# rubiruchi/ofdm_uhd

Measured on AMD Instinct MI355X. Metric: OFDM symbols/sec (TX+loopback RX) @ N_fft=512; packet CRC pass rate, higher is better.
Workload: dtype f32; 1 GPU; N_fft=512, occ=200, QPSK, CP=128, synthetic AWGN channel (BASELINE configs[1]); payload_bytes=1026, symbols_per_packet=22, streams=1, iq_buffers=1, parallelism=independent streams, 1 per GPU

## Files before the change

include/ofdm_hip.h:

```cpp
#ifndef OFDM_HIP_H
#define OFDM_HIP_H

#include <stddef.h>
#include <stdint.h>

#ifdef __cplusplus
extern "C" {
#endif

#define OFDM_ABI_VERSION 6

#define OFDM_MAX_FFT 4096
#define OFDM_MAX_CARRIER_HEX 1024
#define OFDM_MAX_TAPS 512
#define OFDM_MAX_ARITY 256
#define OFDM_MASK_LEN 4096
#define OFDM_MAX_PKT_LEN 4096

enum {
  OFDM_OK = 0,
  OFDM_E_INVAL = -1,
  OFDM_E_NOMEM = -2,
  OFDM_E_CAPACITY = -3,
  OFDM_E_HIP = -4,
// ... 456 lines not shown
int ofdm_ldpc_payload_len(uint32_t coded_len, uint32_t *payload_len);
int ofdm_ldpc_coded_len_rate(uint32_t rate, uint32_t payload_len, uint32_t *coded_len);
int ofdm_ldpc_payload_len_rate(uint32_t rate, uint32_t coded_len, uint32_t *payload_len);
int ofdm_ldpc_encode(ofdm_handle *h, const ofdm_ldpc_cfg *cfg, const uint8_t *payloads, const uint64_t *payload_off,
                     const uint32_t *payload_len, int nblk, uint8_t *coded, uint64_t coded_cap, uint64_t *coded_off);
int ofdm_ldpc_decode(ofdm_handle *h, const ofdm_ldpc_cfg *cfg, const uint8_t *coded, const uint64_t *coded_off,
                     const uint32_t *coded_len, int nblk, uint8_t *payloads, uint64_t payload_cap, uint64_t *payload_off,
                     uint8_t *ok, uint32_t *corrected, uint8_t *iters, uint32_t *cw_failed);
int ofdm_ldpc_decode_soft(ofdm_handle *h, const ofdm_ldpc_cfg *cfg, const int8_t *soft, const uint64_t *soft_off,
                          const uint32_t *coded_len, int nblk, uint8_t *payloads, uint64_t payload_cap,
                          uint64_t *payload_off, uint8_t *ok, uint32_t *corrected, uint8_t *iters, uint32_t *cw_failed);
int ofdm_rx_ldpc_decode_soft(ofdm_handle *h, const ofdm_ldpc_cfg *cfg, uint8_t *payloads, uint64_t payload_cap,
                             uint64_t *payload_off, uint8_t *ok, uint32_t *corrected, uint8_t *iters, uint32_t *cw_failed,
                             int max_pkts, int *n);
int ofdm_ldpc_last_ms(const ofdm_handle *h, double *ms);

int ofdm_rx_set_origin(ofdm_handle *h, uint64_t first_sample_index);
int ofdm_rx_submit(ofdm_handle *h, const ofdm_c32 *iq, uint64_t nsamples);
int ofdm_rx_packet_pos(ofdm_handle *h, uint64_t *pos, int cap, int *n);
int ofdm_rx_nco_state(ofdm_handle *h, uint64_t *flags, uint64_t *phase, double *step, uint8_t *swallowed,
                      int cap, int *n);
int ofdm_rx_set_flag_history(ofdm_handle *h, int enable, int n, const int64_t *flags, const double *steps,
                             const uint8_t *swallowed, int64_t trust_after, int64_t pred_flag, uint64_t pred_phase, double pred_step);

enum {
  OFDM_TAP_TX_PACKETS = 0,
  OFDM_TAP_TX_FREQ = 1,
  OFDM_TAP_RX_CHAN_FILT = 2,
  OFDM_TAP_RX_METRIC = 3,
  OFDM_TAP_RX_PEAKS = 4,
  OFDM_TAP_RX_ANGLES = 5,
  OFDM_TAP_RX_FRAMES = 6,
  OFDM_TAP_RX_FFT = 7,
  OFDM_TAP_RX_ACQ = 8,
  OFDM_TAP_RX_SINK = 9,
  OFDM_TAP_RX_PACKETS = 10,
  OFDM_TAP_TX_MAPPER = 11,
  OFDM_TAP_TX_IFFT = 12,
  OFDM_TAP_RX_SAMPLER = 13,
  OFDM_TAP_RX_SIGMIX = 14,
  OFDM_TAP_RX_NCO = 15,
  OFDM_TAP_RX_PRESEL = 16,
  OFDM_TAP_RX_DEMAPPED = 17,
  OFDM_TAP_RX_RUN_AVG = 18,
  OFDM_TAP_COUNT = 19
};
// ... 27 lines not shown
```

ofdm_uhd_amd/_abi.py:

```python
import ctypes as C
import os

OFDM_ABI_VERSION = 6
OFDM_MAX_FFT = 4096
OFDM_MAX_TAPS = 512
OFDM_MAX_ARITY = 256
OFDM_MASK_LEN = 4096
OFDM_MAX_PKT_LEN = 4096
OFDM_MAX_CARRIER_HEX = 1024
OFDM_DDC_MAX_TAPS = 1024
OFDM_DDC_BANK_MAX_LINKS = 8
OFDM_RESAMP_MAX_TAPS = 1024
OFDM_RESAMP_BANK_MAX_LINKS = 8
OFDM_DUC_MAX_TAPS = 1024
OFDM_DUC_BANK_MAX_LINKS = 8
OFDM_TX_RESAMP_MAX_TAPS = 1024
OFDM_TX_RESAMP_BANK_MAX_LINKS = 8
OFDM_PFB_MAX_CHANNELS = 64
OFDM_PFB_MAX_TAPS = 1024
OFDM_MULTIPATH_MAX_PATHS = 16
OFDM_MULTIPATH_MAX_TONES = 4
OFDM_MULTIPATH_MAX_DELAY = 1023
OFDM_FEC_MAX_PAYLOAD = 2040
OFDM_FEC_MAX_CODED = 4090
# ... 64 lines not shown
        ("fixed_freq_offset", C.c_float),
        ("reserved0", C.c_uint32),
    ]


class ofdm_chan(C.Structure):
    _fields_ = [
        ("sigma", C.c_float),
        ("cfo", C.c_float),
        ("seed", C.c_uint64),
        ("stream_id", C.c_uint64),
        ("lead_samples", C.c_uint64),
        ("tail_samples", C.c_uint64),
    ]


class ofdm_stats(C.Structure):
    _fields_ = [(n, C.c_uint64) for n in (
        "symbols", "samples", "peaks", "frames", "headers_ok", "packets", "crc_ok",
        "chained_frames", "overflow")]

    def as_dict(self):
        return {n: int(getattr(self, n)) for n, _ in self._fields_}


class ofdm_sense_cfg(C.Structure):
    _fields_ = [
        ("struct_size", C.c_uint32),
        ("fft_size", C.c_uint32),
        ("tune_delay", C.c_uint32),
        ("dwell_delay", C.c_uint32),
        ("avg_msgs", C.c_uint32),
        ("skip_msgs", C.c_uint32),
        ("threshold", C.c_double),
        ("window", C.c_float * OFDM_SENSE_MAX_FFT),
    ]


class ofdm_pkt_quality(C.Structure):
    _fields_ = [
        ("flag", C.c_uint64),
        ("first_symbol", C.c_uint32),
        ("nsym", C.c_uint32),
        ("ncarriers", C.c_uint32),
        ("coarse", C.c_int32),
        ("cfo_bins", C.c_float),
# ... 201 lines not shown
    "ofdm_set_rx_iq_format", "ofdm_set_tx_iq_format",
    "ofdm_set_ddc", "ofdm_ddc_reset", "ofdm_ddc_count", "ofdm_ddc", "ofdm_ddc_taps", "ofdm_ddc_last_ms",
    "ofdm_set_duc", "ofdm_duc_reset", "ofdm_duc", "ofdm_duc_last_ms",
    "ofdm_set_ddc_bank", "ofdm_ddc_bank_reset", "ofdm_ddc_bank_count", "ofdm_ddc_bank", "ofdm_ddc_bank_taps",
    "ofdm_ddc_bank_last_ms",
    "ofdm_set_resamp", "ofdm_resamp_reset", "ofdm_resamp_count", "ofdm_resamp", "ofdm_resamp_taps", "ofdm_resamp_last_ms",
    "ofdm_set_resamp_bank", "ofdm_resamp_bank_reset", "ofdm_resamp_bank_count", "ofdm_resamp_bank", "ofdm_resamp_bank_taps",
    "ofdm_resamp_bank_last_ms",
    "ofdm_set_tx_resamp", "ofdm_tx_resamp_reset", "ofdm_tx_resamp_count", "ofdm_tx_resamp", "ofdm_tx_resamp_last_ms",
    "ofdm_set_pfb", "ofdm_pfb_reset", "ofdm_pfb_count", "ofdm_pfb", "ofdm_pfb_last_ms",
    "ofdm_set_pfb_synth", "ofdm_pfb_synth_reset", "ofdm_pfb_synth", "ofdm_pfb_synth_last_ms",
    "ofdm_set_duc_bank", "ofdm_duc_bank_reset", "ofdm_duc_bank", "ofdm_duc_bank_taps", "ofdm_duc_bank_last_ms",
    "ofdm_set_tx_resamp_bank", "ofdm_tx_resamp_bank_reset", "ofdm_tx_resamp_bank_count", "ofdm_tx_resamp_bank",
    "ofdm_tx_resamp_bank_taps", "ofdm_tx_resamp_bank_last_ms",
    "ofdm_set_multipath", "ofdm_multipath_reset", "ofdm_multipath", "ofdm_multipath_last_ms",
    "ofdm_fec_coded_len", "ofdm_fec_payload_len", "ofdm_fec_encode", "ofdm_fec_decode", "ofdm_fec_decode_soft",
    "ofdm_fec_last_ms", "ofdm_fec_coded_len_rate", "ofdm_fec_payload_len_rate", "ofdm_fec_punct_last_ms",
    "ofdm_set_rx_soft", "ofdm_rx_soft", "ofdm_rx_fec_decode_soft", "ofdm_rx_soft_last_ms",
    "ofdm_fec_decode_rel", "ofdm_fec_decode_soft_rel", "ofdm_rx_fec_decode_soft_rel",
    "ofdm_rs_coded_len", "ofdm_rs_payload_len", "ofdm_rs_encode", "ofdm_rs_decode", "ofdm_rs_last_ms",
    "ofdm_rs_decode_rel", "ofdm_rs_rel_from_soft", "ofdm_rs_rel_last_ms",
    "ofdm_ldpc_coded_len", "ofdm_ldpc_payload_len", "ofdm_ldpc_encode", "ofdm_ldpc_decode", "ofdm_ldpc_decode_soft",
    "ofdm_rx_ldpc_decode_soft", "ofdm_ldpc_last_ms", "ofdm_ldpc_coded_len_rate", "ofdm_ldpc_payload_len_rate",
)

_LIB = None
LIB_PATH = os.environ.get("OFDM_HIP_LIB") or os.path.join(os.path.dirname(os.path.abspath(__file__)), "csrc",
                                                         "libofdm_hip.so")


def _declare(lib):
    vp, u8p, u32p, u64p = C.c_void_p, C.c_void_p, C.POINTER(C.c_uint32), C.POINTER(C.c_uint64)
    H = C.c_void_p
    lib.ofdm_abi_version.restype = C.c_int
    lib.ofdm_device_count.restype = C.c_int
    lib.ofdm_create.argtypes = [C.POINTER(ofdm_cfg), C.POINTER(H)]
    lib.ofdm_destroy.argtypes = [H]
    lib.ofdm_destroy.restype = None
    lib.ofdm_last_error.argtypes = [H]
    lib.ofdm_last_error.restype = C.c_char_p
    lib.ofdm_set_stream.argtypes = [H, vp]
    lib.ofdm_set_tx_amplitude.argtypes = [H, C.c_float]
    lib.ofdm_set_carrier_map.argtypes = [H, C.c_char_p]
    lib.ofdm_set_channel.argtypes = [H, C.POINTER(ofdm_chan)]
    lib.ofdm_framed_len.argtypes = [H, C.c_uint32, u32p]
    lib.ofdm_make_packets.argtypes = [H, u8p, u64p, u32p, C.c_int, u8p, C.c_uint64, u64p]
# ... 95 lines not shown
    lib.ofdm_ldpc_coded_len_rate.argtypes = [C.c_uint32, C.c_uint32, u32p]
    lib.ofdm_ldpc_payload_len_rate.argtypes = [C.c_uint32, C.c_uint32, u32p]
    lib.ofdm_ldpc_encode.argtypes = [H, LC, u8p, u64p, u32p, C.c_int, u8p, C.c_uint64, u64p]
    lib.ofdm_ldpc_decode.argtypes = [H, LC, u8p, u64p, u32p, C.c_int, u8p, C.c_uint64, u64p, vp, u32p, vp, u32p]
    lib.ofdm_ldpc_decode_soft.argtypes = lib.ofdm_ldpc_decode.argtypes
    lib.ofdm_rx_ldpc_decode_soft.argtypes = [H, LC, u8p, C.c_uint64, u64p, vp, u32p, vp, u32p, C.c_int, C.POINTER(C.c_int)]
    lib.ofdm_ldpc_last_ms.argtypes = [H, C.POINTER(C.c_double)]
    lib.ofdm_set_taps.argtypes = [H, C.c_uint32]
    lib.ofdm_tap.argtypes = [H, C.c_int, vp, C.c_uint64, u64p]
    lib.ofdm_prof_enable.argtypes = [H, C.c_int]
    lib.ofdm_prof_reset.argtypes = [H]
    lib.ofdm_prof_get.argtypes = [H, C.c_int, C.POINTER(C.c_double), u64p]
    lib.ofdm_kernel_name.argtypes = [C.c_int]
    lib.ofdm_kernel_name.restype = C.c_char_p
    SC = C.POINTER(ofdm_sense_cfg)
    lib.ofdm_sense_count.argtypes = [SC, C.c_uint64, u64p, u64p]
    lib.ofdm_sense.argtypes = [H, SC, vp, C.c_uint64, vp, C.c_uint64, vp, vp, vp, C.c_uint64, u64p, u64p]
    lib.ofdm_sense_decide.argtypes = [H, SC, vp, C.c_uint64, vp, vp, vp, C.c_uint64, u64p]
    lib.ofdm_set_rx_sense.argtypes = [H, SC]
    lib.ofdm_rx_sense_result.argtypes = [H, vp, C.c_uint64, vp, vp, vp, C.c_uint64, u64p, u64p]
    lib.ofdm_rx_packet_pos.argtypes = [H, vp, C.c_int, C.POINTER(C.c_int)]
    lib.ofdm_rx_nco_state.argtypes = [H, vp, vp, vp, vp, C.c_int, C.POINTER(C.c_int)]
    lib.ofdm_rx_set_origin.argtypes = [H, C.c_uint64]
    lib.ofdm_rx_snr.argtypes = [H, C.POINTER(C.c_float)]
    lib.ofdm_set_rx_quality.argtypes = [H, C.c_int]
    lib.ofdm_rx_quality.argtypes = [H, vp, C.c_int, C.POINTER(C.c_int)]
    lib.ofdm_set_rx_csi.argtypes = [H, C.c_int]
    lib.ofdm_rx_csi.argtypes = [H, C.c_int, C.c_int, vp, vp, vp, vp, C.POINTER(C.c_int)]
    lib.ofdm_rx_csi_summary.argtypes = [H, C.c_int, u32p, vp, vp, vp, vp, vp]
    lib.ofdm_rx_submit.argtypes = [H, C.c_void_p, C.c_uint64]
    lib.ofdm_rx_set_flag_history.argtypes = [H, C.c_int, C.c_int, vp, vp, vp, C.c_int64, C.c_int64, C.c_uint64, C.c_double]
    lib.ofdm_sense_device_msgs.argtypes = [H, C.POINTER(C.c_void_p), u64p, u32p]
    lib.ofdm_sense_redecide.argtypes = [H, SC]
    for name in EXPORTS:
        fn = getattr(lib, name)
        if fn.restype is C.c_int and name not in ("ofdm_abi_version", "ofdm_device_count"):
            pass
    return lib


def _preload_hip_runtime():
    try:
        import importlib.util
        spec = importlib.util.find_spec("torch")
        if spec is None or not spec.origin:
            return
# ... 22 lines not shown
```

ofdm_uhd_amd/csrc/engine_rx.inc:

```

template <typename T>
static int dev_excl_scan(ofdm_handle* h, const T* d_in, uint64_t n, T* d_out, T* d_total) {
  const uint64_t nb = (n + SCAN_BLOCK - 1) / SCAN_BLOCK;
  HIPCHK(h, h->rx.partial.ensure(sizeof(T) * std::max<uint64_t>(nb, 1)));
  T* part = h->rx.partial.as<T>();
  if (n == 0) {
    if (d_total) HIPCHK(h, hipMemsetAsync(d_total, 0, sizeof(T), h->stream));
    return OFDM_OK;
  }
  hipLaunchKernelGGL(HIP_KERNEL_NAME(k_scan_partials<T>), dim3((unsigned)nb), dim3(256), 0, h->stream, d_in, n, part);
  hipLaunchKernelGGL(HIP_KERNEL_NAME(k_scan_top<T>), dim3(1), dim3(256), 0, h->stream, part, nb, d_total);
  hipLaunchKernelGGL(HIP_KERNEL_NAME(k_scan_final<T>), dim3((unsigned)nb), dim3(256), 0, h->stream, d_in, n, part, d_out);
  HIPCHK(h, hipGetLastError());
  return OFDM_OK;
}

template <int N, bool TWL, bool TAPS, bool CSI = false>
static int launch_demod_t(ofdm_handle* h, const DemodParams& q, size_t shmem) {
  constexpr int T = N / 8, FPW = demod_fpw(N);
  if (shmem > 64 * 1024)
    HIPCHK(h, hipFuncSetAttribute(reinterpret_cast<const void*>(&k_rx_demod<N, TWL, TAPS, CSI>),
                                  hipFuncAttributeMaxDynamicSharedMemorySize, (int)shmem));
  hipLaunchKernelGGL(HIP_KERNEL_NAME(k_rx_demod<N, TWL, TAPS, CSI>), dim3((q.nframes + FPW - 1) / FPW), dim3(T * FPW), shmem,
                     h->stream, q);
  HIPCHK(h, hipGetLastError());
  return OFDM_OK;
}
template <int N, bool TWL>
static int launch_demod_v(ofdm_handle* h, const DemodParams& q, size_t shmem) {
  if (q.csi_eq) return launch_demod_t<N, TWL, true, true>(h, q, shmem);
  const bool instr = q.tap_mode != 0 || q.tap_sampler || q.tap_fft || q.tap_acq || q.tap_sink || q.tap_demapped || q.qual;
  return instr ? launch_demod_t<N, TWL, true>(h, q, shmem) : launch_demod_t<N, TWL, false>(h, q, shmem);
}

template <int N>
static int launch_demod(ofdm_handle* h, const DemodParams& q0) {
  DemodParams q = q0;
  constexpr int T = N / 8, WAVES = demod_fpw(N) * ((T + WAVE - 1) / WAVE);
  const bool grid = q.grid != nullptr;
  const bool csi = q.csi_eq != nullptr;
  auto bytes = [&](bool twl, bool sm) {
    return (size_t)demod_lds_bytes(N, twl, sm, q.occ, q.arity, q.nmap, q.nbits, q.shift, grid, csi);
  };
  constexpr int CU_WAVES = 4 * demod_waves_per_simd(N);
  auto wgs = [&](size_t b) { return std::max<size_t>(1, std::min<size_t>(std::max(1, CU_WAVES / WAVES), CU_LDS_BYTES / b)); };
  constexpr bool base_twl = !fft_onebuf(N);
  const size_t w0 = wgs(bytes(base_twl, false));
  bool twl = base_twl;
  if constexpr (fft_onebuf(N)) twl = wgs(bytes(true, false)) == w0 && bytes(true, false) <= CU_LDS_BYTES;
  q.smap_lds = (wgs(bytes(twl, true)) == w0 && bytes(twl, true) <= CU_LDS_BYTES) ? 1 : 0;
  if (const char* e = getenv("OFDM_DEMOD_LDS")) {
    const int v = atoi(e);
    if constexpr (fft_onebuf(N)) twl = (v & 1) != 0;
    q.smap_lds = (v >> 1) & 1;
  }
  const size_t shmem = bytes(twl, q.smap_lds != 0);
  if (shmem > CU_LDS_BYTES) FAIL(h, OFDM_E_INVAL, "configuration needs more than 160 KiB of LDS in k_rx_demod");
  if constexpr (fft_onebuf(N)) {
    return twl ? launch_demod_v<N, true>(h, q, shmem) : launch_demod_v<N, false>(h, q, shmem);
  } else {
    return launch_demod_v<N, true>(h, q, shmem);
  }
}

static int run_demod(ofdm_handle* h, const DemodParams& q) {
  switch (h->N) {
    case 64: return launch_demod<64>(h, q);
    case 128: return launch_demod<128>(h, q);
    case 256: return launch_demod<256>(h, q);
    case 512: return launch_demod<512>(h, q);
    case 1024: return launch_demod<1024>(h, q);
    case 2048: return launch_demod<2048>(h, q);
    default: return launch_demod<4096>(h, q);
  }
}

enum { CT_CAND = 0, CT_OVERFLOW = 1, CT_NLO = 2, CT_NHI = 3, CT_CHAIN = 4, CT_NPEAKS = 5, CT_NSYM = 6, CT_KEYTOT = 7,
       CT_DEFR = 8 , CT_RAWTOT = 13, CT_PIECES = 14, CT_STASH = 15, CT_RECS = 16, CT_COUNT = 17 };

static int sync_params(ofdm_handle* h, uint64_t nsamples, bool cap_full, SyncParams* out) {
  RxState& rx = h->rx;
  const int N = h->N, CP = h->CP, T = SYNC_TILE;
  const uint64_t ntiles = (nsamples + T - 1) / T;
  const int tiles_per_seg = 32 * ((N + CP + T - 1) / T);
  const uint64_t egrid = std::min<uint64_t>(ntiles, 256ull * 8ull), egrid_small = std::min<uint64_t>(ntiles, 256ull * 16ull);
  const uint64_t cand_cap = (cap_full ? nsamples + nsamples / 8 : nsamples / 16) + (egrid + 16) * SYNC_CHUNK_C + egrid_small * 2048ull;
  const uint64_t piece_cap = (cap_full ? nsamples / 2 + 1 : nsamples / 128) + (egrid + egrid_small + 16) * SYNC_CHUNK_P;
  HIPCHK(h, rx.y.ensure(nsamples * sizeof(c32)));
  HIPCHK(h, rx.tile_B.ensure(ntiles * sizeof(double)));
  HIPCHK(h, rx.tile_np.ensure(ntiles * sizeof(uint32_t)));
  HIPCHK(h, rx.tile_pieces.ensure(piece_cap * sizeof(SyncPiece)));
  HIPCHK(h, rx.tile_first.ensure(ntiles * sizeof(uint64_t)));
  HIPCHK(h, rx.avg_in.ensure(ntiles * sizeof(double)));
  HIPCHK(h, rx.cand_u.ensure(cand_cap * sizeof(float)));
  HIPCHK(h, rx.cand_P.ensure(cand_cap * sizeof(c32)));
  HIPCHK(h, rx.counters.ensure(CT_COUNT * sizeof(uint64_t)));
  HIPCHK(h, rx.counts.ensure(ntiles * sizeof(uint32_t)));
// ... 1357 lines not shown
```

ofdm_uhd_amd/csrc/fft.h:

```cpp
#pragma once
#include "common.h"

__host__ __device__ constexpr int fft_lds_points(int n) { return n + n / 8; }
__host__ __device__ constexpr bool fft_onebuf(int n) { return n >= 2048; }
__host__ __device__ constexpr int fft_lds_bufs(int n) { return fft_onebuf(n) ? 1 : 2; }
__host__ __device__ constexpr int fft_lds_bytes(int n) { return fft_lds_bufs(n) * fft_lds_points(n) * (int)sizeof(c32); }

__device__ __forceinline__ int lpad(int i) { return i + (i >> 3); }

struct FftWaveSync {
  __device__ __forceinline__ void operator()() const {
    __builtin_amdgcn_fence(__ATOMIC_RELEASE, "wavefront");
    __builtin_amdgcn_wave_barrier();
    __builtin_amdgcn_fence(__ATOMIC_ACQUIRE, "wavefront");
  }
};
struct FftBlockSync {
  __device__ __forceinline__ void operator()() const { __syncthreads(); }
};

template <bool INV>
__device__ __forceinline__ c32 mul_mi(c32 a) {
  return INV ? mk(-a.im, a.re) : mk(a.im, -a.re);
}
// ... 290 lines not shown
    fft_pass_tw<2048, 8, 4, INV, false, false, true, SyncFn, TwFn, PK>(e, t, A, A, tw, sync);
    sync();
    fft_pass_tw<2048, 8, 32, INV, false, false, true, SyncFn, TwFn, PK>(e, t, A, A, tw, sync);
    sync();
    fft_pass_tw<2048, 8, 256, INV, false, true, false, SyncFn, TwFn, PK>(e, t, A, nullptr, tw, sync);
  } else {
    static_assert(N == 4096, "unsupported FFT length");
    (void)B;
    fft_pass_tw<4096, 8, 1, INV, true, false, false, SyncFn, TwFn, PK>(e, t, nullptr, A, tw, sync);
    sync();
    fft_pass_tw<4096, 8, 8, INV, false, false, true, SyncFn, TwFn, PK>(e, t, A, A, tw, sync);
    sync();
    fft_pass_tw<4096, 8, 64, INV, false, false, true, SyncFn, TwFn, PK>(e, t, A, A, tw, sync);
    sync();
    fft_pass_tw<4096, 8, 512, INV, false, true, false, SyncFn, TwFn, PK>(e, t, A, nullptr, tw, sync);
  }
}

template <int N, bool INV, typename SyncFn, bool PK = false>
__device__ __forceinline__ void fft_run(c32 e[8], int t, c32* lds, const c32* __restrict__ tw, SyncFn sync) {
  fft_run_tw<N, INV, SyncFn, PK, FftTwTable>(e, t, lds, FftTwTable{tw}, sync);
}

template <int N, bool INV, bool PK = false, typename SyncFn = int, typename TwFn = FftTwTable>
__device__ __forceinline__ void fft_run1(c32 e[8], int t, c32* A, const TwFn& tw, SyncFn sync) {
  sync();
  if constexpr (N == 64) {
    fft_pass_tw<64, 8, 1, INV, true, false, false, SyncFn, TwFn, PK>(e, t, nullptr, A, tw, sync);
    sync();
    fft_pass_tw<64, 8, 8, INV, false, true, false, SyncFn, TwFn, PK>(e, t, A, nullptr, tw, sync);
  } else if constexpr (N == 128) {
    fft_pass_tw<128, 2, 1, INV, true, false, false, SyncFn, TwFn, PK>(e, t, nullptr, A, tw, sync);
    sync();
    fft_pass_tw<128, 8, 2, INV, false, false, true, SyncFn, TwFn, PK>(e, t, A, A, tw, sync);
    sync();
    fft_pass_tw<128, 8, 16, INV, false, true, false, SyncFn, TwFn, PK>(e, t, A, nullptr, tw, sync);
  } else if constexpr (N == 256) {
    fft_pass_tw<256, 4, 1, INV, true, false, false, SyncFn, TwFn, PK>(e, t, nullptr, A, tw, sync);
    sync();
    fft_pass_tw<256, 8, 4, INV, false, false, true, SyncFn, TwFn, PK>(e, t, A, A, tw, sync);
    sync();
    fft_pass_tw<256, 8, 32, INV, false, true, false, SyncFn, TwFn, PK>(e, t, A, nullptr, tw, sync);
  } else if constexpr (N == 512) {
    fft_pass_tw<512, 8, 1, INV, true, false, false, SyncFn, TwFn, PK>(e, t, nullptr, A, tw, sync);
    sync();
    fft_pass_tw<512, 8, 8, INV, false, false, true, SyncFn, TwFn, PK>(e, t, A, A, tw, sync);
    sync();
    fft_pass_tw<512, 8, 64, INV, false, true, false, SyncFn, TwFn, PK>(e, t, A, nullptr, tw, sync);
// ... 13 lines not shown
```

ofdm_uhd_amd/csrc/rx_demod.h:

```cpp
#pragma once
#include "common.h"
#include "fft.h"
#ifndef DEMOD_PK
#define DEMOD_PK true
#endif
#include "host_util.h"

#define RAW_SLOT 4096

enum { FR_BAD_HEADER = 0, FR_COMPLETE = 1, FR_INCOMPLETE = 2 };

struct FrameResult {
  uint32_t status;
  uint32_t packetlen;
  uint32_t end_frame;
  uint32_t header_ok;
};

struct FrameQuality {
  float pilot, null_;
  float err, ref;
  uint32_t nsym;
  int32_t coarse;
  uint64_t first_symbol;
// ... 136 lines not shown
  FrameQuality* qual;
  c32* csi_eq;
  float* csi_pre;
  float* csi_err;
  float* csi_ref;
  int csi_stride;
};

__host__ __device__ inline int demod_symbits_words(int nmap, int nbits) { return (nmap * nbits + 8 + 31) / 32 + 2; }
__host__ __device__ inline int demod_hinv_len(int n, int occ, int shift) {
  const int need = (occ + 2 * shift + 2 + 1) / 2;
  return need > occ ? need : occ;
}
__host__ __device__ inline int demod_red_floats(int n) { return n / 8 == WAVE ? 0 : 64; }
#ifndef DEMOD_FPW
#define DEMOD_FPW 4
#endif
__host__ __device__ constexpr int demod_fpw(int n) { return n / 8 == WAVE ? DEMOD_FPW : 1; }
__host__ __device__ inline int demod_lds_shared(int n, bool twl, bool smap_lds, int arity, int nmap, bool grid) {
  const int b = (twl ? fft_tw_lds_points(n) : 0) * (int)sizeof(c32) + arity * (int)sizeof(c32) +
                (grid ? (int)sizeof(SlicerGrid) : 0) + (smap_lds ? ((nmap * 2 + 3) & ~3) : 0);
  return (b + 15) & ~15;
}
__host__ __device__ inline int demod_lds_frame(int n, int occ, int nmap, int nbits, int shift, bool csi = false) {
  const int b = fft_lds_points(n) * (int)sizeof(c32) + (demod_hinv_len(n, occ, shift) + occ) * (int)sizeof(c32) +
                demod_red_floats(n) * (int)sizeof(float) + ((demod_symbits_words(nmap, nbits) + 3) & ~3) * 4 +
                (csi ? 2 * occ * (int)sizeof(float) : 0);
  return (b + 15) & ~15;
}
__host__ __device__ inline int demod_lds_bytes(int n, bool twl, bool smap_lds, int occ, int arity, int nmap, int nbits, int shift,
                                               bool grid, bool csi = false) {
  return demod_lds_shared(n, twl, smap_lds, arity, nmap, grid) + demod_fpw(n) * demod_lds_frame(n, occ, nmap, nbits, shift, csi);
}

__device__ __forceinline__ void wave_sum2_tree(float& a, float& b) {
  float t0, t1;
  asm volatile(
      "v_mov_b32 %2, %0\n\t"
      "v_mov_b32 %3, %1\n\t"
      "s_nop 1\n\t"
      "v_permlane32_swap_b32 %0, %2\n\t"
      "v_permlane32_swap_b32 %1, %3\n\t"
      "s_nop 1\n\t"
      "v_add_f32 %0, %0, %2\n\t"
      "v_add_f32 %1, %1, %3\n\t"
      "v_mov_b32 %2, %0\n\t"
      "v_mov_b32 %3, %1\n\t"
      "s_nop 1\n\t"
      "v_permlane16_swap_b32 %0, %2\n\t"
      "v_permlane16_swap_b32 %1, %3\n\t"
      "s_nop 1\n\t"
      "v_add_f32 %0, %0, %2\n\t"
      "v_add_f32 %1, %1, %3\n\t"
      "s_nop 1\n\t"
      "v_add_f32_dpp %2, %0, %0 row_shl:8 row_mask:0xf bank_mask:0x3\n\t"
// ... 114 lines not shown
}

#ifdef SYNC_STAMPS
__device__ unsigned long long g_demod_stamps[16];
#define DSTAMP(i)                                                        \
  do {                                                                   \
    if (threadIdx.x == 0) {                                              \
      __builtin_amdgcn_s_waitcnt(0xC07F);                                \
      const unsigned long long now_ = __builtin_amdgcn_s_memtime();     \
      __builtin_amdgcn_s_waitcnt(0xC07F);                                \
      dst_acc[i] += now_ - dst_last;                                     \
      dst_last = now_;                                                   \
    }                                                                    \
  } while (0)
#else
#define DSTAMP(i) do { } while (0)
#endif
#ifndef DEMOD_WAVES
#define DEMOD_WAVES 4
#endif
#ifndef DEMOD_WAVES_BIG
#define DEMOD_WAVES_BIG 4
#endif
__host__ __device__ constexpr int demod_waves_per_simd(int n) { return (n / 8 >= 256) ? DEMOD_WAVES_BIG : DEMOD_WAVES; }
template <int FPW>
__device__ __forceinline__ void frame_sync() {
  if constexpr (FPW > 1) {
    FftWaveSync()();
  } else {
    __syncthreads();
  }
}
template <int N, bool TWL, bool INSTR, bool CSI = false>
__global__ void __launch_bounds__(((N / 8 < 64) ? 64 : N / 8) * demod_fpw(N), demod_waves_per_simd(N)) k_rx_demod(DemodParams q_in) {
  static_assert(INSTR || !CSI, "the CSI instantiation is an instrumented one");
  DemodParams q = q_in;
  if constexpr (!INSTR) {
    q.tap_sampler = nullptr;
    q.tap_fft = nullptr;
    q.tap_acq = nullptr;
    q.tap_sink = nullptr;
    q.tap_demapped = nullptr;
    q.tap_mode = 0;
    q.qual = nullptr;
  }
  static_assert(TWL || fft_onebuf(N), "up to N = 1024 the twiddles are always in LDS");
  constexpr int T = N / 8;
  constexpr int FPW = demod_fpw(N);
  extern __shared__ __align__(16) unsigned char smem[];
  const bool use_grid = q.grid != nullptr;
  c32* twl = reinterpret_cast<c32*>(smem);
  c32* cst = twl + (TWL ? fft_tw_lds_points(N) : 0);
  SlicerGrid* grid = reinterpret_cast<SlicerGrid*>(cst + q.arity);
  int16_t* smapL = reinterpret_cast<int16_t*>(reinterpret_cast<unsigned char*>(grid) + (q.grid ? sizeof(SlicerGrid) : 0));
  const int slot = FPW > 1 ? __builtin_amdgcn_readfirstlane((int)(threadIdx.x / T)) : 0;
  unsigned char* mine = smem + demod_lds_shared(N, TWL, q.smap_lds != 0, q.arity, q.nmap, use_grid) +
                        slot * demod_lds_frame(N, q.occ, q.nmap, q.nbits, q.shift, CSI);
  c32* fftbuf = reinterpret_cast<c32*>(mine);
  c32* Ysh = fftbuf;
  c32* hinv = fftbuf + fft_lds_points(N);
  float* sd = reinterpret_cast<float*>(hinv);
  c32* dfe = hinv + demod_hinv_len(N, q.occ, q.shift);
  float* red = reinterpret_cast<float*>(dfe + q.occ);
  uint32_t* sbits = reinterpret_cast<uint32_t*>(red + demod_red_floats(N));
  const int sbw = demod_symbits_words(q.nmap, q.nbits);
  float* csi_acc = reinterpret_cast<float*>(sbits + ((sbw + 3) & ~3));

  const int t = FPW > 1 ? (int)(threadIdx.x % T) : (int)threadIdx.x;
  const uint32_t f = blockIdx.x * FPW + (uint32_t)slot;
  const uint32_t q_nframes = dyn_nframes(q.dyn, q.nframes), q_j0 = dyn_j0(q.dyn, q.j0);

  {
    const int nthr = FPW * T, th = threadIdx.x;
    for (int i = th; i < q.arity; i += nthr) cst[i] = q.constellation[i];
    if constexpr (TWL)
      for (int i = th; i < fft_tw_used(N); i += nthr) twl[lpad(i)] = q.tw[i];
    if (q.smap_lds)
      for (int i = th; i < q.nmap; i += nthr) smapL[i] = q.smap[i];
    if (use_grid)
      for (int i = th; i < (int)(sizeof(SlicerGrid) / 4); i += nthr)
        reinterpret_cast<uint32_t*>(grid)[i] = reinterpret_cast<const uint32_t*>(q.grid)[i];
  }
  __syncthreads();
// ... 87 lines not shown
        }
      } else {
#pragma unroll
        for (int m = 0; m < 8; m++) {
          const uint64_t n = s00 + (uint64_t)(tl + m * T);
          int64_t i = (int64_t)j;
          while (i >= 0 && q.peaks[i] > n) i--;
          double ph = 0.0;
          if (i >= 0)
            ph = q.Phi[i] + q.step[i] * (double)(n - q.peaks[i] + 1);
          else if (q.ref_on)
            ph = q.ref_phi + q.ref_step * (double)((int64_t)n - q.ref_peak + 1);
          const dc r = dexpj(ph);
          e[m] = cmul(e[m], mk((float)r.re, (float)r.im));
        }
      }
      DSTAMP(1);
      if (q.tap_sampler) {
#pragma unroll
        for (int m = 0; m < 8; m++) q.tap_sampler[(symb + k) * (uint64_t)N + (uint64_t)(tl + m * T)] = e[m];
      }
      if constexpr (!fft_onebuf(N)) {
        if constexpr (FPW > 1)
          fft_run1<N, false, DEMOD_PK, FftWaveSync, FftTwLds>(e, tl, fftbuf, FftTwLds{twl}, FftWaveSync());
        else
          fft_run1<N, false, DEMOD_PK, FftBlockSync, FftTwLds>(e, tl, fftbuf, FftTwLds{twl}, FftBlockSync());
      } else if constexpr (TWL) {
        fft_run_tw<N, false, FftBlockSync, DEMOD_PK, FftTwLds>(e, tl, fftbuf, FftTwLds{twl}, FftBlockSync());
      } else {
        fft_run<N, false, FftBlockSync, DEMOD_PK>(e, tl, fftbuf, q.tw, FftBlockSync());
      }
      DSTAMP(2);
      if (k < K) {
        const uint64_t s1 = s00 + (uint64_t)(k + 1) * (uint64_t)q.L;
#pragma unroll
        for (int m = 0; m < 8; m++) nx[m] = q.y[s1 + (uint64_t)(tl + m * T)];
      }
      frame_sync<FPW>();
#pragma unroll
      for (int m = 0; m < 8; m++) Ysh[(tl + m * T + N / 2) & (N - 1)] = e[m];
      frame_sync<FPW>();
      if (q.tap_fft) {
#pragma unroll
        for (int m = 0; m < 8; m++) q.tap_fft[(symb + k) * (uint64_t)N + (uint64_t)(tl + m * T)] = Ysh[tl + m * T];
      }

      DSTAMP(3);
      if (k == 0) {
        phase_count = 1;
        const int sbase = q.zl - q.shift, slen = q.occ + 2 * q.shift;
        for (int r = t; r < slen; r += T) {
          const int i = sbase + r;
          float v = 0.f;
          if (i >= 0 && i < N - 2) v = cnorm(csub(Ysh[i], Ysh[i + 2]));
          sd[r] = v;
        }
        frame_sync<FPW>();
        int index = 0;
        float mx = 0.f;
        for (int i0 = q.zl - q.shift; i0 < q.zl + q.shift; i0 += 2) {
          float pa = 0.f, pb = 0.f;
          for (int jj = t; jj < q.occ; jj += T) {
            const float kdv = q.kd[jj];
            const int ra = i0 - sbase + jj;
            pa = pa + kdv * sd[ra];
            pb = pb + kdv * sd[ra + 1];
          }
          block_sum2_f<T>(pa, pb, red);
          if (pa > mx) {
            mx = pa;
            index = i0;
          }
          if (i0 + 1 < q.zl + q.shift && pb > mx) {
            mx = pb;
            index = i0 + 1;
          }
        }
        coarse = __builtin_amdgcn_readfirstlane(index - q.zl);
        {
          const double a = -6.283185307179586476925 * (double)coarse * (double)q.CP / (double)N * 1.0;
          const float af = (float)a;
          c32 comp;
          det_sincosf(af, &comp.im, &comp.re);
          for (int i = 2 * t; i < q.occ; i += 2 * T) {
            const int yi = i + q.zl + coarse;
            const c32 Y = (yi >= 0 && yi < N) ? Ysh[yi] : mk(0.f, 0.f);
            hinv[i] = cdiv(q.ks[i], cmul(comp, Y));
          }
          frame_sync<FPW>();
          for (int i = 2 * t + 1; i < q.occ; i += 2 * T) {
            if (i + 1 < q.occ) {
              const c32 a1 = hinv[i + 1], a0 = hinv[i - 1];
              hinv[i] = mk((a1.re + a0.re) / 2.0f, (a1.im + a0.im) / 2.0f);
            }
          }
          frame_sync<FPW>();
          if (t == 0 && !(q.occ & 1)) hinv[q.occ - 1] = hinv[q.occ - 2];
          frame_sync<FPW>();
        }
        if constexpr (INSTR) if (qon && cf == f) {
          for (int i = t; i < q.occ; i += T) {
            const int yi = i + q.zl + coarse;
            const c32 Y = (yi >= 0 && yi < N) ? Ysh[yi] : mk(0.f, 0.f);
            const c32 kv = q.ks[i];
            const float p2 = cnorm(Y);
            if (kv.re != 0.f || kv.im != 0.f)
              q_pil = q_pil + p2;
            else
              q_nul = q_nul + p2;
// ... 35 lines not shown

      DSTAMP(4);
      if (done) {
        frame_sync<FPW>();
        continue;
      }
      if (sstate == 0) {
        sstate = 1;
        frame_sync<FPW>();
        continue;
      }
      c32 carrier;
      det_sincosf(pll_phase, &carrier.im, &carrier.re);
      carrier = mk(f32_uniform(carrier.re), f32_uniform(carrier.im));
      float are = 0.f, aim = 0.f;
      const uint32_t carry_bits = nbits_total & 7u;
      for (int c = t; c < q.nmap; c += T) {
        int i;
        if (q.smap_lds)
          i = ((const __attribute__((address_space(3))) int16_t*)smapL)[c];
        else
          i = ((const __attribute__((address_space(1))) int16_t*)q.smap)[c];
        const int yi = i + q.zl + coarse;
        const c32 Y = (yi >= 0 && yi < N) ? Ysh[yi] : mk(0.f, 0.f);
        const c32 in = cmul(cmul(hinv[i], comp), Y);
        const c32 sigrot = cmul(cmul(in, carrier), dfe[c]);
        unsigned best = 0;
        float bestd;
        const float sre = fabsf(sigrot.re), sim = fabsf(sigrot.im);
        if (q.sign_kind != 0 && sre > q.sign_eps && sre < q.sign_bound && sim < q.sign_bound &&
            (q.sign_kind == 1 || sim > q.sign_eps)) {
          const bool rp = sigrot.re > 0.0f, ip = sigrot.im > 0.0f;
          if (q.sign_kind == 1)
            best = rp ? sidx1 : sidx0;
          else
            best = rp ? (ip ? sidx3 : sidx2) : (ip ? sidx1 : sidx0);
        } else if (use_grid && sre <= grid->bound && sim <= grid->bound) {
          int ka = 0, kb = 0;
          for (int a = 1; a < grid->nr - 1; a++) ka += (sigrot.re >= grid->lr[a]) ? 1 : 0;
          for (int b = 1; b < grid->ni - 1; b++) kb += (sigrot.im >= grid->li[b]) ? 1 : 0;
          best = grid->idx[ka * grid->ni + kb];
          bestd = cnorm(csub(sigrot, cst[best]));
#pragma unroll
          for (int c4 = 1; c4 < 4; c4++) {
            const unsigned cand = grid->idx[(ka + (c4 >> 1)) * grid->ni + kb + (c4 & 1)];
            const float dd = cnorm(csub(sigrot, cst[cand]));
            if (dd < bestd || (dd == bestd && cand < best)) {
// ... 132 lines not shown
```

Measured before the change: 131.4 million OFDM symbols/s.

## Add compact-LDS demod variant for N=512 with single-plane FFT exchange

Adds a COMPACT instantiation of the RX demod kernel for N=512 that does the FFT data exchange one float plane at a time (real parts, then imaginary parts) in a half-size buffer. After the FFT it keeps only the occupied-plus-shift bins in Ysh, re-storing them when the coarse offset falls outside the window. This shrinks per-frame LDS and raises the launch-bounds wave target from 4 to 5 per SIMD, aiming for more workgroups per CU. In exchange the FFT exchange needs extra barriers and memory round-trips, and the index bookkeeping is more involved. It also adds a host plan query API and an env override to turn the variant off.

Result: no change. 132.7 million OFDM symbols/s, median of 6 (+1.0%).

```diff
diff --git a/include/ofdm_hip.h b/include/ofdm_hip.h
--- a/include/ofdm_hip.h
+++ b/include/ofdm_hip.h
@@ -502,6 +502,16 @@
                       int cap, int *n);
 int ofdm_rx_set_flag_history(ofdm_handle *h, int enable, int n, const int64_t *flags, const double *steps,
                              const uint8_t *swallowed, int64_t trust_after, int64_t pred_flag, uint64_t pred_phase, double pred_step);
+typedef struct {
+  uint32_t lds_bytes;
+  int32_t compact;
+  int32_t twiddles_lds;
+  int32_t map_lds;
+  int32_t frames_per_wg;
+  int32_t wgs_per_cu;
+} ofdm_demod_plan;
+int ofdm_rx_demod_plan(int fft_length, int occupied_tones, int nmap, int nbits, int arity, int grid, int shift,
+                       int instrumented, int csi, ofdm_demod_plan *out);
 
 enum {
   OFDM_TAP_TX_PACKETS = 0,
diff --git a/ofdm_uhd_amd/_abi.py b/ofdm_uhd_amd/_abi.py
--- a/ofdm_uhd_amd/_abi.py
+++ b/ofdm_uhd_amd/_abi.py
@@ -110,6 +110,11 @@
 
     def as_dict(self):
         return {n: int(getattr(self, n)) for n, _ in self._fields_}
+
+
+class ofdm_demod_plan(C.Structure):
+    _fields_ = [("lds_bytes", C.c_uint32), ("compact", C.c_int32), ("twiddles_lds", C.c_int32), ("map_lds", C.c_int32),
+                ("frames_per_wg", C.c_int32), ("wgs_per_cu", C.c_int32)]
 
 
 class ofdm_sense_cfg(C.Structure):
@@ -357,6 +362,7 @@
     "ofdm_rs_decode_rel", "ofdm_rs_rel_from_soft", "ofdm_rs_rel_last_ms",
     "ofdm_ldpc_coded_len", "ofdm_ldpc_payload_len", "ofdm_ldpc_encode", "ofdm_ldpc_decode", "ofdm_ldpc_decode_soft",
     "ofdm_rx_ldpc_decode_soft", "ofdm_ldpc_last_ms", "ofdm_ldpc_coded_len_rate", "ofdm_ldpc_payload_len_rate",
+    "ofdm_rx_demod_plan",
 )
 
 _LIB = None
@@ -498,6 +504,7 @@
     lib.ofdm_rx_packet_pos.argtypes = [H, vp, C.c_int, C.POINTER(C.c_int)]
     lib.ofdm_rx_nco_state.argtypes = [H, vp, vp, vp, vp, C.c_int, C.POINTER(C.c_int)]
     lib.ofdm_rx_set_origin.argtypes = [H, C.c_uint64]
+    lib.ofdm_rx_demod_plan.argtypes = [C.c_int] * 9 + [C.POINTER(ofdm_demod_plan)]
     lib.ofdm_rx_snr.argtypes = [H, C.POINTER(C.c_float)]
     lib.ofdm_set_rx_quality.argtypes = [H, C.c_int]
     lib.ofdm_rx_quality.argtypes = [H, vp, C.c_int, C.POINTER(C.c_int)]
diff --git a/ofdm_uhd_amd/csrc/engine_rx.inc b/ofdm_uhd_amd/csrc/engine_rx.inc
--- a/ofdm_uhd_amd/csrc/engine_rx.inc
+++ b/ofdm_uhd_amd/csrc/engine_rx.inc
@@ -15,51 +15,79 @@
   return OFDM_OK;
 }
 
-template <int N, bool TWL, bool TAPS, bool CSI = false>
+template <int N, bool TWL, bool TAPS, bool CSI = false, bool COMPACT = false>
 static int launch_demod_t(ofdm_handle* h, const DemodParams& q, size_t shmem) {
   constexpr int T = N / 8, FPW = demod_fpw(N);
   if (shmem > 64 * 1024)
-    HIPCHK(h, hipFuncSetAttribute(reinterpret_cast<const void*>(&k_rx_demod<N, TWL, TAPS, CSI>),
+    HIPCHK(h, hipFuncSetAttribute(reinterpret_cast<const void*>(&k_rx_demod<N, TWL, TAPS, CSI, COMPACT>),
                                   hipFuncAttributeMaxDynamicSharedMemorySize, (int)shmem));
-  hipLaunchKernelGGL(HIP_KERNEL_NAME(k_rx_demod<N, TWL, TAPS, CSI>), dim3((q.nframes + FPW - 1) / FPW), dim3(T * FPW), shmem,
-                     h->stream, q);
+  hipLaunchKernelGGL(HIP_KERNEL_NAME(k_rx_demod<N, TWL, TAPS, CSI, COMPACT>), dim3((q.nframes + FPW - 1) / FPW), dim3(T * FPW),
+                     shmem, h->stream, q);
   HIPCHK(h, hipGetLastError());
   return OFDM_OK;
 }
+static bool demod_instr(const DemodParams& q) {
+  return q.csi_eq || q.tap_mode != 0 || q.tap_sampler || q.tap_fft || q.tap_acq || q.tap_sink || q.tap_demapped || q.qual;
+}
 template <int N, bool TWL>
-static int launch_demod_v(ofdm_handle* h, const DemodParams& q, size_t shmem) {
+static int launch_demod_v(ofdm_handle* h, const DemodParams& q, size_t shmem, bool compact) {
   if (q.csi_eq) return launch_demod_t<N, TWL, true, true>(h, q, shmem);
-  const bool instr = q.tap_mode != 0 || q.tap_sampler || q.tap_fft || q.tap_acq || q.tap_sink || q.tap_demapped || q.qual;
-  return instr ? launch_demod_t<N, TWL, true>(h, q, shmem) : launch_demod_t<N, TWL, false>(h, q, shmem);
-}
-
+  if (demod_instr(q)) return launch_demod_t<N, TWL, true>(h, q, shmem);
+  if constexpr (demod_compact_fits(N, 0, 0)) {
+    if (compact) return launch_demod_t<N, TWL, false, false, true>(h, q, shmem);
+  }
+  return launch_demod_t<N, TWL, false>(h, q, shmem);
+}
+
+struct DemodShape {
+  int occ, arity, nmap, nbits, shift;
+  bool grid, csi, instr;
+};
+struct DemodLaunch {
+  bool twl, smap_lds, compact;
+  size_t shmem;
+  int wgs_per_cu;
+};
+template <int N>
+static DemodLaunch demod_launch_plan(const DemodShape& q) {
+  constexpr int T = N / 8, WAVES = demod_fpw(N) * ((T + WAVE - 1) / WAVE);
+  const bool grid = q.grid, csi = q.csi;
+  bool compact = !q.instr && !q.csi && demod_compact_fits(N, q.occ, q.shift);
+  if (const char* e = getenv("OFDM_DEMOD_COMPACT"))
+    if (atoi(e) == 0) compact = false;
+  auto bytes = [&](bool twl, bool sm) {
+    return (size_t)demod_lds_bytes(N, twl, sm, q.occ, q.arity, q.nmap, q.nbits, q.shift, grid, csi, compact);
+  };
+  const int CU_WAVES = 4 * demod_waves_per_simd(N, compact);
+  auto wgs = [&](size_t b) { return std::max<size_t>(1, std::min<size_t>(std::max(1, CU_WAVES / WAVES), CU_LDS_BYTES / b)); };
+  constexpr bool base_twl = !fft_onebuf(N);
+  const size_t w0 = wgs(bytes(base_twl, false));
+  DemodLaunch p;
+  p.compact = compact;
+  p.twl = base_twl;
+  if constexpr (fft_onebuf(N)) p.twl = wgs(bytes(true, false)) == w0 && bytes(true, false) <= CU_LDS_BYTES;
+  p.smap_lds = wgs(bytes(p.twl, true)) == w0 && bytes(p.twl, true) <= CU_LDS_BYTES;
+  if (const char* e = getenv("OFDM_DEMOD_LDS")) {
+    const int v = atoi(e);
+    if constexpr (fft_onebuf(N)) p.twl = (v & 1) != 0;
+    p.smap_lds = ((v >> 1) & 1) != 0;
+  }
+  if (compact) p.smap_lds = true;
+  p.shmem = bytes(p.twl, p.smap_lds);
+  p.wgs_per_cu = p.shmem <= CU_LDS_BYTES ? (int)wgs(p.shmem) : 0;
+  return p;
+}
 template <int N>
 static int launch_demod(ofdm_handle* h, const DemodParams& q0) {
   DemodParams q = q0;
-  constexpr int T = N / 8, WAVES = demod_fpw(N) * ((T + WAVE - 1) / WAVE);
-  const bool grid = q.grid != nullptr;
-  const bool csi = q.csi_eq != nullptr;
-  auto bytes = [&](bool twl, bool sm) {
-    return (size_t)demod_lds_bytes(N, twl, sm, q.occ, q.arity, q.nmap, q.nbits, q.shift, grid, csi);
-  };
-  constexpr int CU_WAVES = 4 * demod_waves_per_simd(N);
-  auto wgs = [&](size_t b) { return std::max<size_t>(1, std::min<size_t>(std::max(1, CU_WAVES / WAVES), CU_LDS_BYTES / b)); };
-  constexpr bool base_twl = !fft_onebuf(N);
-  const size_t w0 = wgs(bytes(base_twl, false));
-  bool twl = base_twl;
-  if constexpr (fft_onebuf(N)) twl = wgs(bytes(true, false)) == w0 && bytes(true, false) <= CU_LDS_BYTES;
-  q.smap_lds = (wgs(bytes(twl, true)) == w0 && bytes(twl, true) <= CU_LDS_BYTES) ? 1 : 0;
-  if (const char* e = getenv("OFDM_DEMOD_LDS")) {
-    const int v = atoi(e);
-    if constexpr (fft_onebuf(N)) twl = (v & 1) != 0;
-    q.smap_lds = (v >> 1) & 1;
-  }
-  const size_t shmem = bytes(twl, q.smap_lds != 0);
-  if (shmem > CU_LDS_BYTES) FAIL(h, OFDM_E_INVAL, "configuration needs more than 160 KiB of LDS in k_rx_demod");
+  const DemodLaunch p = demod_launch_plan<N>(
+      DemodShape{q.occ, q.arity, q.nmap, q.nbits, q.shift, q.grid != nullptr, q.csi_eq != nullptr, demod_instr(q)});
+  q.smap_lds = p.smap_lds ? 1 : 0;
+  if (p.shmem > CU_LDS_BYTES) FAIL(h, OFDM_E_INVAL, "configuration needs more than 160 KiB of LDS in k_rx_demod");
   if constexpr (fft_onebuf(N)) {
-    return twl ? launch_demod_v<N, true>(h, q, shmem) : launch_demod_v<N, false>(h, q, shmem);
+    return p.twl ? launch_demod_v<N, true>(h, q, p.shmem, p.compact) : launch_demod_v<N, false>(h, q, p.shmem, p.compact);
   } else {
-    return launch_demod_v<N, true>(h, q, shmem);
+    return launch_demod_v<N, true>(h, q, p.shmem, p.compact);
   }
 }
 
@@ -73,6 +101,32 @@
     case 2048: return launch_demod<2048>(h, q);
     default: return launch_demod<4096>(h, q);
   }
+}
+
+extern "C" int ofdm_rx_demod_plan(int fft_length, int occupied_tones, int nmap, int nbits, int arity, int grid, int shift,
+                                  int instrumented, int csi, ofdm_demod_plan* out) {
+  if (!out || occupied_tones < 1 || occupied_tones > fft_length || nmap < 0 || nmap > occupied_tones || nbits < 1 ||
+      nbits > 8 || arity != (1 << nbits) || shift < 0)
+    return OFDM_E_INVAL;
+  const DemodShape q{occupied_tones, arity, nmap, nbits, shift, grid != 0, csi != 0, instrumented != 0 || csi != 0};
+  DemodLaunch p;
+  switch (fft_length) {
+    case 64: p = demod_launch_plan<64>(q); break;
+    case 128: p = demod_launch_plan<128>(q); break;
+    case 256: p = demod_launch_plan<256>(q); break;
+    case 512: p = demod_launch_plan<512>(q); break;
+    case 1024: p = demod_launch_plan<1024>(q); break;
+    case 2048: p = demod_launch_plan<2048>(q); break;
+    case 4096: p = demod_launch_plan<4096>(q); break;
+    default: return OFDM_E_INVAL;
+  }
+  out->lds_bytes = (uint32_t)p.shmem;
+  out->compact = p.compact;
+  out->twiddles_lds = p.twl;
+  out->map_lds = p.smap_lds;
+  out->frames_per_wg = demod_fpw(fft_length);
+  out->wgs_per_cu = p.wgs_per_cu;
+  return OFDM_OK;
 }
 
 enum { CT_CAND = 0, CT_OVERFLOW = 1, CT_NLO = 2, CT_NHI = 3, CT_CHAIN = 4, CT_NPEAKS = 5, CT_NSYM = 6, CT_KEYTOT = 7,
diff --git a/ofdm_uhd_amd/csrc/fft.h b/ofdm_uhd_amd/csrc/fft.h
--- a/ofdm_uhd_amd/csrc/fft.h
+++ b/ofdm_uhd_amd/csrc/fft.h
@@ -336,8 +336,93 @@
   fft_run_tw<N, INV, SyncFn, PK, FftTwTable>(e, t, lds, FftTwTable{tw}, sync);
 }
 
-template <int N, bool INV, bool PK = false, typename SyncFn = int, typename TwFn = FftTwTable>
+template <int N, int R, int LS, bool INV, typename TwFn, bool PK>
+__device__ __forceinline__ void fft_bfly(c32 v[R], int k, const TwFn& twf) {
+  if constexpr (PK) {
+    cv pv[R];
+#pragma unroll
+    for (int q = 0; q < R; q++) pv[q] = cv_of(v[q]);
+    if constexpr (LS > 1) {
+#pragma unroll
+      for (int q = 1; q < R; q++) pv[q] = pk_cmul_tw<INV>(pv[q], cv_of(twf.template fwd<N, LS, R>(k, q)));
+    }
+    if constexpr (R == 8) {
+      dft8_pk<INV>(pv);
+    } else if constexpr (R == 4) {
+      dft4_pk<INV>(pv[0], pv[1], pv[2], pv[3]);
+    } else {
+      const cv sm = pv[0] + pv[1], df = pv[0] - pv[1];
+      pv[0] = sm;
+      pv[1] = df;
+    }
+#pragma unroll
+    for (int q = 0; q < R; q++) v[q] = c32_of(pv[q]);
+  } else {
+    if constexpr (LS > 1) {
+#pragma unroll
+      for (int q = 1; q < R; q++) v[q] = cmul_f(v[q], twf.template get<N, LS, R, INV>(k, q));
+    }
+    if constexpr (R == 8) {
+      dft8<INV>(v);
+    } else if constexpr (R == 4) {
+      dft4<INV>(v[0], v[1], v[2], v[3]);
+    } else {
+      dft2(v[0], v[1]);
+    }
+  }
+}
+
+template <int LS, bool IM>
+__device__ __forceinline__ void fft_plane_put(const c32 x[8], int t, float* F) {
+  const int k = (LS == 1) ? 0 : (t % LS);
+  const int wbase = lpad((t - k) * 8 + k);
+#pragma unroll
+  for (int r = 0; r < 8; r++) F[wbase + r * LS + ((r * LS) >> 3)] = IM ? x[r].im : x[r].re;
+}
+template <int N, bool IM>
+__device__ __forceinline__ void fft_plane_get(c32 x[8], int t, const float* F) {
+  constexpr int STRIDE = N / 8;
+  static_assert(STRIDE % 8 == 0, "padded read offsets need STRIDE % 8 == 0");
+  const int rbase = lpad(t);
+#pragma unroll
+  for (int q = 0; q < 8; q++) {
+    const float v = F[rbase + q * (STRIDE + STRIDE / 8)];
+    if (IM)
+      x[q].im = v;
+    else
+      x[q].re = v;
+  }
+}
+template <int N, int LS, typename SyncFn>
+__device__ __forceinline__ void fft_plane_exchange(c32 x[8], int t, float* F, SyncFn sync) {
+  fft_plane_put<LS, false>(x, t, F);
+  sync();
+  fft_plane_get<N, false>(x, t, F);
+  sync();
+  fft_plane_put<LS, true>(x, t, F);
+  sync();
+  fft_plane_get<N, true>(x, t, F);
+}
+template <int N, bool INV, bool PK, typename SyncFn, typename TwFn>
+__device__ __forceinline__ void fft_run1_plane(c32 e[8], int t, float* F, const TwFn& tw, SyncFn sync) {
+  static_assert(N == 64 || N == 512, "single-plane exchange: radix-8 passes only");
+  sync();
+  fft_bfly<N, 8, 1, INV, TwFn, PK>(e, 0, tw);
+  fft_plane_exchange<N, 1>(e, t, F, sync);
+  if constexpr (N == 512) {
+    fft_bfly<N, 8, 8, INV, TwFn, PK>(e, t % 8, tw);
+    sync();
+    fft_plane_exchange<N, 8>(e, t, F, sync);
+  }
+  fft_bfly<N, 8, N / 8, INV, TwFn, PK>(e, t, tw);
+}
+
+template <int N, bool INV, bool PK = false, typename SyncFn = int, typename TwFn = FftTwTable, bool PLANE = false>
 __device__ __forceinline__ void fft_run1(c32 e[8], int t, c32* A, const TwFn& tw, SyncFn sync) {
+  if constexpr (PLANE) {
+    fft_run1_plane<N, INV, PK, SyncFn, TwFn>(e, t, reinterpret_cast<float*>(A), tw, sync);
+    return;
+  }
   sync();
   if constexpr (N == 64) {
     fft_pass_tw<64, 8, 1, INV, true, false, false, SyncFn, TwFn, PK>(e, t, nullptr, A, tw, sync);
diff --git a/ofdm_uhd_amd/csrc/rx_demod.h b/ofdm_uhd_amd/csrc/rx_demod.h
--- a/ofdm_uhd_amd/csrc/rx_demod.h
+++ b/ofdm_uhd_amd/csrc/rx_demod.h
@@ -182,15 +182,25 @@
                 (grid ? (int)sizeof(SlicerGrid) : 0) + (smap_lds ? ((nmap * 2 + 3) & ~3) : 0);
   return (b + 15) & ~15;
 }
+__host__ __device__ constexpr int demod_ysh_bins(int occ, int shift) { return occ + 2 * shift + 2; }
+__host__ __device__ constexpr bool demod_compact_fits(int n, int occ, int shift) {
+  return n == 512 && shift >= 0 && demod_ysh_bins(occ, shift) * (int)sizeof(c32) <= fft_lds_points(n) * (int)sizeof(float) &&
+         (n - occ + 1) / 2 - shift >= 0 && (n - occ + 1) / 2 - shift + demod_ysh_bins(occ, shift) <= n;
+}
 __host__ __device__ inline int demod_lds_frame(int n, int occ, int nmap, int nbits, int shift, bool csi = false) {
   const int b = fft_lds_points(n) * (int)sizeof(c32) + (demod_hinv_len(n, occ, shift) + occ) * (int)sizeof(c32) +
                 demod_red_floats(n) * (int)sizeof(float) + ((demod_symbits_words(nmap, nbits) + 3) & ~3) * 4 +
                 (csi ? 2 * occ * (int)sizeof(float) : 0);
   return (b + 15) & ~15;
 }
+__host__ __device__ inline int demod_lds_frame_compact(int n, int occ, int nmap, int nbits, int shift) {
+  return demod_lds_frame(n, occ, nmap, nbits, shift) - fft_lds_points(n) * (int)(sizeof(c32) - sizeof(float));
+}
 __host__ __device__ inline int demod_lds_bytes(int n, bool twl, bool smap_lds, int occ, int arity, int nmap, int nbits, int shift,
-                                               bool grid, bool csi = false) {
-  return demod_lds_shared(n, twl, smap_lds, arity, nmap, grid) + demod_fpw(n) * demod_lds_frame(n, occ, nmap, nbits, shift, csi);
+                                               bool grid, bool csi = false, bool compact = false) {
+  return demod_lds_shared(n, twl, smap_lds, arity, nmap, grid) +
+         demod_fpw(n) * (compact ? demod_lds_frame_compact(n, occ, nmap, nbits, shift)
+                                 : demod_lds_frame(n, occ, nmap, nbits, shift, csi));
 }
 
 __device__ __forceinline__ void wave_sum2_tree(float& a, float& b) {
@@ -351,7 +361,12 @@
 #ifndef DEMOD_WAVES_BIG
 #define DEMOD_WAVES_BIG 4
 #endif
-__host__ __device__ constexpr int demod_waves_per_simd(int n) { return (n / 8 >= 256) ? DEMOD_WAVES_BIG : DEMOD_WAVES; }
+#ifndef DEMOD_WAVES_COMPACT
+#define DEMOD_WAVES_COMPACT 5
+#endif
+__host__ __device__ constexpr int demod_waves_per_simd(int n, bool compact = false) {
+  return compact ? DEMOD_WAVES_COMPACT : (n / 8 >= 256) ? DEMOD_WAVES_BIG : DEMOD_WAVES;
+}
 template <int FPW>
 __device__ __forceinline__ void frame_sync() {
   if constexpr (FPW > 1) {
@@ -360,9 +375,12 @@
     __syncthreads();
   }
 }
-template <int N, bool TWL, bool INSTR, bool CSI = false>
-__global__ void __launch_bounds__(((N / 8 < 64) ? 64 : N / 8) * demod_fpw(N), demod_waves_per_simd(N)) k_rx_demod(DemodParams q_in) {
+template <int N, bool TWL, bool INSTR, bool CSI = false, bool COMPACT = false>
+__global__ void __launch_bounds__(((N / 8 < 64) ? 64 : N / 8) * demod_fpw(N), demod_waves_per_simd(N, COMPACT))
+k_rx_demod(DemodParams q_in) {
   static_assert(INSTR || !CSI, "the CSI instantiation is an instrumented one");
+  static_assert(!COMPACT || (!INSTR && demod_fpw(N) > 1 && demod_compact_fits(N, 0, 0)),
+                "the compact frame serves the lean one-wave kernel: no symbol tap reads the whole spectrum there");
   DemodParams q = q_in;
   if constexpr (!INSTR) {
     q.tap_sampler = nullptr;
@@ -373,6 +391,7 @@
     q.tap_mode = 0;
     q.qual = nullptr;
   }
+  if constexpr (COMPACT) q.smap_lds = 1;
   static_assert(TWL || fft_onebuf(N), "up to N = 1024 the twiddles are always in LDS");
   constexpr int T = N / 8;
   constexpr int FPW = demod_fpw(N);
@@ -385,9 +404,13 @@
   const int slot = FPW > 1 ? __builtin_amdgcn_readfirstlane((int)(threadIdx.x / T)) : 0;
   unsigned char* mine = smem + demod_lds_shared(N, TWL, q.smap_lds != 0, q.arity, q.nmap, use_grid) +
                         slot * demod_lds_frame(N, q.occ, q.nmap, q.nbits, q.shift, CSI);
+  if constexpr (COMPACT)
+    mine = smem + demod_lds_shared(N, TWL, q.smap_lds != 0, q.arity, q.nmap, use_grid) +
+           slot * demod_lds_frame_compact(N, q.occ, q.nmap, q.nbits, q.shift);
   c32* fftbuf = reinterpret_cast<c32*>(mine);
   c32* Ysh = fftbuf;
-  c32* hinv = fftbuf + fft_lds_points(N);
+  static_assert(fft_lds_points(N) * sizeof(float) % 16 == 0, "the single-plane buffer keeps a frame's 16-byte alignment");
+  c32* hinv = fftbuf + (COMPACT ? fft_lds_points(N) / 2 : fft_lds_points(N));
   float* sd = reinterpret_cast<float*>(hinv);
   c32* dfe = hinv + demod_hinv_len(N, q.occ, q.shift);
   float* red = reinterpret_cast<float*>(dfe + q.occ);
@@ -521,7 +544,7 @@
       }
       if constexpr (!fft_onebuf(N)) {
         if constexpr (FPW > 1)
-          fft_run1<N, false, DEMOD_PK, FftWaveSync, FftTwLds>(e, tl, fftbuf, FftTwLds{twl}, FftWaveSync());
+          fft_run1<N, false, DEMOD_PK, FftWaveSync, FftTwLds, COMPACT>(e, tl, fftbuf, FftTwLds{twl}, FftWaveSync());
         else
           fft_run1<N, false, DEMOD_PK, FftBlockSync, FftTwLds>(e, tl, fftbuf, FftTwLds{twl}, FftBlockSync());
       } else if constexpr (TWL) {
@@ -536,8 +559,18 @@
         for (int m = 0; m < 8; m++) nx[m] = q.y[s1 + (uint64_t)(tl + m * T)];
       }
       frame_sync<FPW>();
-#pragma unroll
-      for (int m = 0; m < 8; m++) Ysh[(tl + m * T + N / 2) & (N - 1)] = e[m];
+      if constexpr (COMPACT) {
+        const int ybase = k == 0 ? q.zl - q.shift : q.zl + coarse;
+        const unsigned ylen = k == 0 ? (unsigned)demod_ysh_bins(q.occ, q.shift) : (unsigned)q.occ;
+#pragma unroll
+        for (int m = 0; m < 8; m++) {
+          const unsigned r = (unsigned)(((tl + m * T + N / 2) & (N - 1)) - ybase);
+          if (r < ylen) Ysh[r] = e[m];
+        }
+      } else {
+#pragma unroll
+        for (int m = 0; m < 8; m++) Ysh[(tl + m * T + N / 2) & (N - 1)] = e[m];
+      }
       frame_sync<FPW>();
       if (q.tap_fft) {
 #pragma unroll
@@ -551,7 +584,10 @@
         for (int r = t; r < slen; r += T) {
           const int i = sbase + r;
           float v = 0.f;
-          if (i >= 0 && i < N - 2) v = cnorm(csub(Ysh[i], Ysh[i + 2]));
+          if constexpr (COMPACT)
+            v = cnorm(csub(Ysh[r], Ysh[r + 2]));
+          else if (i >= 0 && i < N - 2)
+            v = cnorm(csub(Ysh[i], Ysh[i + 2]));
           sd[r] = v;
         }
         frame_sync<FPW>();
@@ -576,6 +612,19 @@
           }
         }
         coarse = __builtin_amdgcn_readfirstlane(index - q.zl);
+        int yoff = q.shift + coarse;
+        if constexpr (COMPACT) {
+          if (coarse < -q.shift || sstate != 0) {
+            yoff = 0;
+            frame_sync<FPW>();
+#pragma unroll
+            for (int m = 0; m < 8; m++) {
+              const unsigned r = (unsigned)(((tl + m * T + N / 2) & (N - 1)) - (q.zl + coarse));
+              if (r < (unsigned)q.occ) Ysh[r] = e[m];
+            }
+            frame_sync<FPW>();
+          }
+        }
         {
           const double a = -6.283185307179586476925 * (double)coarse * (double)q.CP / (double)N * 1.0;
           const float af = (float)a;
@@ -583,7 +632,7 @@
           det_sincosf(af, &comp.im, &comp.re);
           for (int i = 2 * t; i < q.occ; i += 2 * T) {
             const int yi = i + q.zl + coarse;
-            const c32 Y = (yi >= 0 && yi < N) ? Ysh[yi] : mk(0.f, 0.f);
+            const c32 Y = COMPACT ? Ysh[yoff + i] : (yi >= 0 && yi < N) ? Ysh[yi] : mk(0.f, 0.f);
             hinv[i] = cdiv(q.ks[i], cmul(comp, Y));
           }
           frame_sync<FPW>();
@@ -665,7 +714,7 @@
         else
           i = ((const __attribute__((address_space(1))) int16_t*)q.smap)[c];
         const int yi = i + q.zl + coarse;
-        const c32 Y = (yi >= 0 && yi < N) ? Ysh[yi] : mk(0.f, 0.f);
+        const c32 Y = COMPACT ? Ysh[i] : (yi >= 0 && yi < N) ? Ysh[yi] : mk(0.f, 0.f);
         const c32 in = cmul(cmul(hinv[i], comp), Y);
         const c32 sigrot = cmul(cmul(in, carrier), dfe[c]);
         unsigned best = 0;
```
